# lucasnewman/f5-tts-mlx

Measured on NVIDIA H100. Metric: mel-frames/sec, higher is better.
Workload: dtype bf16

## Files before the change

f5_tts_mlx_b200/csrc/attention.cu:

```cuda
#include "attention_sm90.cuh"
#include "host_common.h"

static int attention_impl(const void* qkv, int64_t ld_qkv, void* out, int64_t ld_out, int32_t batch, int32_t frames,
                          int32_t heads, int32_t head_dim, const int32_t* kv_len, int out_fp8, void* stream_,
                          float* scale_out = nullptr);

extern "C" int f5_attention_fwd(const void* qkv, int64_t ld_qkv, void* out, int64_t ld_out,
                                int32_t batch, int32_t frames, int32_t heads, int32_t head_dim,
                                const int32_t* kv_len, void* stream_) {
  return attention_impl(qkv, ld_qkv, out, ld_out, batch, frames, heads, head_dim, kv_len, 0, stream_);
}
extern "C" int f5_attention_fwd_e4m3(const void* qkv, int64_t ld_qkv, void* out, int64_t ld_out,
                                     int32_t batch, int32_t frames, int32_t heads, int32_t head_dim,
                                     const int32_t* kv_len, void* stream_) {
  return attention_impl(qkv, ld_qkv, out, ld_out, batch, frames, heads, head_dim, kv_len, 1, stream_);
}
extern "C" int f5_attention_fwd_e4m3_scaled(const void* qkv, int64_t ld_qkv, void* out, int64_t ld_out,
                                            int32_t batch, int32_t frames, int32_t heads, int32_t head_dim,
                                            const int32_t* kv_len, float* scale_out, void* stream_) {
  F5_REQUIRE(scale_out != nullptr, "f5_attention_fwd_e4m3_scaled: null scale_out");
  return attention_impl(qkv, ld_qkv, out, ld_out, batch, frames, heads, head_dim, kv_len, 1, stream_, scale_out);
}

static int attention_impl(const void* qkv, int64_t ld_qkv, void* out, int64_t ld_out, int32_t batch, int32_t frames,
                          int32_t heads, int32_t head_dim, const int32_t* kv_len, int out_fp8, void* stream_,
                          float* scale_out) {
  using namespace f5;
  if (int e = device_check()) return e;
  F5_REQUIRE(qkv && out, "f5_attention_fwd: null pointer");
  F5_REQUIRE(head_dim == 64, "f5_attention_fwd: head_dim %d unsupported (only 64)", head_dim);
  F5_REQUIRE(batch > 0 && frames > 0 && heads > 0, "f5_attention_fwd: bad shape");
  F5_REQUIRE(ld_qkv % 8 == 0 && ld_qkv >= 3 * heads * 64, "f5_attention_fwd: bad ld_qkv");
  F5_REQUIRE(ld_out % (out_fp8 ? 16 : 8) == 0 && ld_out >= heads * 64, "f5_attention_fwd: bad ld_out");
  CUtensorMap tm;
  uint64_t dims[3] = {(uint64_t)3 * heads * 64, (uint64_t)frames, (uint64_t)batch};
  uint64_t str[2] = {(uint64_t)ld_qkv * 2, (uint64_t)ld_qkv * 2 * (uint64_t)frames};
  uint32_t box[3] = {64, 128, 1};
  if (int e = make_tmap_bf16(&tm, qkv, 3, dims, str, box)) return e;
  AttnParams p;
  p.B = batch; p.N = frames; p.H = heads;
  p.kv_len = kv_len;
  p.out = reinterpret_cast<__nv_bfloat16*>(out);
  p.ldo = (int)ld_out;
  p.out_fp8 = out_fp8;
  p.scale_out = scale_out;
  cudaStream_t stream = reinterpret_cast<cudaStream_t>(stream_);
  ProfScope ps(PROF_ATTN, 4.0 * batch * heads * (double)frames * frames * 64.0,
               2.0 * batch * (double)frames * heads * 64.0 * 4.0);
  p.prof = ps.slot;
  auto launch = [&](auto kern, SmemAttrOnce& once, dim3 grid, int threads, int smem) -> int {
    F5_CHECK_CUDA(ensure_dyn_smem(once, kern, smem));
    F5_CHECK_CUDA(launch_kernel(kern, grid, dim3(threads), smem, stream, tm, p));
    F5_CHECK_CUDA(cudaGetLastError());
    return 0;
  };
  const dim3 grid(cdiv(frames, 128), heads, batch);
  static SmemAttrOnce o4, o8, o8s;
  if (scale_out != nullptr) return launch(attn_fwd_kernel<true, true>, o8s, grid, 384, AttnSmem::kTotal);
  if (out_fp8) return launch(attn_fwd_kernel<true>, o8, grid, 384, AttnSmem::kTotal);
  return launch(attn_fwd_kernel<false>, o4, grid, 384, AttnSmem::kTotal);
}
```

f5_tts_mlx_b200/csrc/attention_sm90.cuh:

```cuda
#pragma once
#include "ptx.cuh"

namespace f5 {

struct AttnParams {
  int B, N, H;
  const int* kv_len;
  __nv_bfloat16* out;
  int ldo;
  unsigned long long* prof;
  int out_fp8;
  float* scale_out;
};

struct AttnSmem {
  static constexpr int kQ = 0;
  static constexpr int kK = 16384;
  static constexpr int kV = kK + 2 * 16384;
  static constexpr int kBar = kV + 2 * 16384;
  static constexpr int kNumBars = 9;
  static constexpr int kTotal = kBar + kNumBars * 8 + 1024;
};

template <bool kOut8, bool kScaled = false>
__global__ void __launch_bounds__(384, 1)
attn_fwd_kernel(const __grid_constant__ CUtensorMap tma_qkv, const AttnParams p) {
  extern __shared__ uint8_t smem_raw[];
  uint8_t* smem = smem_raw + ((1024u - (smem_u32(smem_raw) & 1023u)) & 1023u);
  uint64_t* bars = reinterpret_cast<uint64_t*>(smem + AttnSmem::kBar);
  uint64_t* q_full = bars + 0;
  uint64_t* k_full = bars + 1;
  uint64_t* k_empty = bars + 3;
  uint64_t* v_full = bars + 5;
  uint64_t* v_empty = bars + 7;

  const int warp = threadIdx.x >> 5, lane = threadIdx.x & 31;
  const int q0 = blockIdx.x * 128;
  const int h = blockIdx.y;
  const int b = blockIdx.z;
  const int HD = p.H * 64;

  if (warp == 0 && elect_one()) {
    tma_prefetch_desc(&tma_qkv);
    mbar_init(q_full, 1);
    for (int i = 0; i < 2; ++i) {
      mbar_init(&k_full[i], 1);
      mbar_init(&k_empty[i], 256);
      mbar_init(&v_full[i], 1);
      mbar_init(&v_empty[i], 256);
    }
    fence_mbar_init();
  }
  __syncthreads();
  pdl_wait();
  if (threadIdx.x == 128) prof_stamp_begin(p.prof);
  int kv_len = p.kv_len ? p.kv_len[b] : p.N;
  kv_len = min(max(kv_len, 1), p.N);
  const int num_kv = (kv_len + 127) >> 7;

  if (warp < 4) {
    if (warp == 0 && elect_one()) {
      mbar_expect_tx(q_full, 16384);
      tma_load_3d(smem + AttnSmem::kQ, &tma_qkv, q_full, h * 64, q0, b);
      for (int j = 0; j < num_kv; ++j) {
        const int s = j & 1;
        const uint32_t ph = (j >> 1) & 1;
        mbar_wait(&k_empty[s], ph ^ 1);
        mbar_expect_tx(&k_full[s], 16384);
        tma_load_3d(smem + AttnSmem::kK + s * 16384, &tma_qkv, &k_full[s], HD + h * 64, j * 128, b);
        mbar_wait(&v_empty[s], ph ^ 1);
        mbar_expect_tx(&v_full[s], 16384);
        tma_load_3d(smem + AttnSmem::kV + s * 16384, &tma_qkv, &v_full[s], 2 * HD + h * 64, j * 128, b);
      }
    }
  } else {
    const int wg = (threadIdx.x >> 7) - 1;
    const int rw = ((threadIdx.x >> 5) & 3) * 16 + (lane >> 2);
    const uint32_t sQ = smem_u32(smem + AttnSmem::kQ) + wg * (64 * 128);
    constexpr float kLog2e = 1.4426950408889634f;
    float o[32];
#pragma unroll
    for (int i = 0; i < 32; ++i) o[i] = 0.f;
    float m_run[2] = {-INFINITY, -INFINITY}, l_run[2] = {0.f, 0.f};
    mbar_wait(q_full, 0);

    for (int j = 0; j < num_kv; ++j) {
      const int s = j & 1;
      const uint32_t ph = (j >> 1) & 1;
      float sv[64];
      mbar_wait(&k_full[s], ph);
      const uint32_t sK = smem_u32(smem + AttnSmem::kK + s * 16384);
      wgmma_fence();
#pragma unroll
      for (int k = 0; k < 4; ++k)
        wgmma_bf16_ss_n128(sv, gmma_desc_sw128(sQ + 32 * k, 16, 1024), gmma_desc_sw128(sK + 32 * k, 16, 1024), k != 0);
      wgmma_commit();
      wgmma_wait<0>();
      wgmma_reg_fence(sv);
      mbar_arrive(&k_empty[s]);

      const int kv0 = j * 128;
      if (kv0 + 128 > kv_len) {
#pragma unroll
        for (int i = 0; i < 64; ++i)
          if (kv0 + 8 * (i >> 2) + 2 * (lane & 3) + (i & 1) >= kv_len) sv[i] = -INFINITY;
      }
      float mx[2] = {m_run[0], m_run[1]};
#pragma unroll
      for (int i = 0; i < 64; ++i) mx[(i >> 1) & 1] = fmaxf(mx[(i >> 1) & 1], sv[i]);
#pragma unroll
      for (int r = 0; r < 2; ++r) {
        mx[r] = fmaxf(mx[r], __shfl_xor_sync(0xffffffffu, mx[r], 1));
        mx[r] = fmaxf(mx[r], __shfl_xor_sync(0xffffffffu, mx[r], 2));
      }
      float sc[2], mb[2];
#pragma unroll
      for (int r = 0; r < 2; ++r) {
        sc[r] = ex2_approx((m_run[r] - mx[r]) * kLog2e);
        m_run[r] = mx[r];
        mb[r] = mx[r] * kLog2e;
        l_run[r] *= sc[r];
      }
#pragma unroll
      for (int i = 0; i < 32; ++i) o[i] *= sc[(i >> 1) & 1];
      uint32_t pa[8][4];
#pragma unroll
      for (int kk = 0; kk < 8; ++kk) {
#pragma unroll
        for (int m = 0; m < 4; ++m) {
          const int i = 8 * kk + 2 * m, r = m & 1;
          const float e0 = ex2_approx(fmaf(sv[i], kLog2e, -mb[r]));
          const float e1 = ex2_approx(fmaf(sv[i + 1], kLog2e, -mb[r]));
          l_run[r] += e0 + e1;
          pa[kk][m] = pack_bf16x2(e0, e1);
        }
      }

      mbar_wait(&v_full[s], ph);
      const uint32_t sV = smem_u32(smem + AttnSmem::kV + s * 16384);
      wgmma_fence();
#pragma unroll
      for (int kk = 0; kk < 8; ++kk) wgmma_bf16_rs_n64_tb(o, pa[kk], gmma_desc_sw128(sV + kk * 2048, 16384, 1024));
      wgmma_commit();
      wgmma_wait<0>();
      wgmma_reg_fence(o);
      mbar_arrive(&v_empty[s]);
    }

    pdl_launch_dependents();
#pragma unroll
    for (int r = 0; r < 2; ++r) {
      l_run[r] += __shfl_xor_sync(0xffffffffu, l_run[r], 1);
      l_run[r] += __shfl_xor_sync(0xffffffffu, l_run[r], 2);
    }
    const float inv[2] = {1.f / l_run[0], 1.f / l_run[1]};
    float qs[2] = {1.f, 1.f}, qinv[2] = {1.f, 1.f};
    if constexpr (kScaled) {
#pragma unroll
      for (int r = 0; r < 2; ++r) {
        float amax = 0.f;
#pragma unroll
        for (int c = 0; c < 8; ++c)
          amax = fmax_nan(amax, fmax_nan(fabsf(o[4 * c + 2 * r] * inv[r]), fabsf(o[4 * c + 2 * r + 1] * inv[r])));
        amax = fmax_nan(amax, __shfl_xor_sync(0xffffffffu, amax, 1));
        amax = fmax_nan(amax, __shfl_xor_sync(0xffffffffu, amax, 2));
        qs[r] = e4m3_block_scale(amax, qinv[r]);
      }
    }
#pragma unroll
    for (int r = 0; r < 2; ++r) {
      const int n = q0 + wg * 64 + rw + 8 * r;
      if (n >= p.N) continue;
      const size_t row = (size_t)b * p.N + n;
      if (kScaled && (lane & 3) == 0) p.scale_out[(size_t)h * p.B * p.N + row] = qs[r];
#pragma unroll
      for (int c = 0; c < 8; ++c) {
        const int col = h * 64 + 8 * c + 2 * (lane & 3);
        float v0 = o[4 * c + 2 * r] * inv[r], v1 = o[4 * c + 2 * r + 1] * inv[r];
        if constexpr (kScaled) { v0 *= qinv[r]; v1 *= qinv[r]; }
        if constexpr (kOut8) {
          uint16_t w;
          asm("cvt.rn.satfinite.e4m3x2.f32 %0, %1, %2;" : "=h"(w) : "f"(v1), "f"(v0));
          *reinterpret_cast<uint16_t*>(reinterpret_cast<uint8_t*>(p.out) + row * p.ldo + col) = w;
        } else {
          *reinterpret_cast<uint32_t*>(p.out + row * p.ldo + col) = pack_bf16x2(v0, v1);
        }
      }
    }
  }

  __syncthreads();
  if (threadIdx.x == 0) prof_stamp_end(p.prof);
}

}
```

f5_tts_mlx_b200/csrc/host_common.h:

```cpp
#pragma once
#include <cuda.h>
#include <cuda_runtime.h>
#include <stdarg.h>
#include <stdint.h>
#include <stdio.h>

#include "../../include/f5_b200.h"

namespace f5 {

int set_error(int code, const char* fmt, ...);

#define F5_CHECK_CUDA(expr)                                                              \
  do {                                                                                   \
    cudaError_t _e = (expr);                                                             \
    if (_e != cudaSuccess)                                                               \
      return f5::set_error(F5_ERR_CUDA, "%s failed: %s (%s:%d)", #expr,                  \
                           cudaGetErrorString(_e), __FILE__, __LINE__);                  \
  } while (0)

#define F5_REQUIRE(cond, ...)                                        \
  do {                                                               \
    if (!(cond)) return f5::set_error(F5_ERR_INVALID, __VA_ARGS__);  \
  } while (0)

int device_check();

int make_tmap_bf16(CUtensorMap* map, const void* base, int rank, const uint64_t* dims,
                   const uint64_t* strides_bytes, const uint32_t* box);
int make_tmap_u8(CUtensorMap* map, const void* base, int rank, const uint64_t* dims,
                 const uint64_t* strides_bytes, const uint32_t* box);
int make_tmap_u8_sw64(CUtensorMap* map, const void* base, int rank, const uint64_t* dims,
                      const uint64_t* strides_bytes, const uint32_t* box);
int make_tmap_out(CUtensorMap* map, const void* base, int elem_bytes, uint64_t cols, uint64_t rows, uint64_t batches,
                  uint64_t ld_elems);

inline int cdiv(int a, int b) { return (a + b - 1) / b; }

int sm_count();

template <typename... KArgs, typename... Args>
inline cudaError_t launch_kernel(void (*kern)(KArgs...), dim3 grid, dim3 block, size_t smem,
                                 cudaStream_t st, Args&&... args) {
  cudaLaunchConfig_t cfg = {};
  cfg.gridDim = grid;
  cfg.blockDim = block;
  cfg.dynamicSmemBytes = smem;
  cfg.stream = st;
  cudaLaunchAttribute attr[1];
  attr[0].id = cudaLaunchAttributeProgrammaticStreamSerialization;
  attr[0].val.programmaticStreamSerializationAllowed = 1;
  cfg.attrs = attr;
  cfg.numAttrs = 1;
  return cudaLaunchKernelEx(&cfg, kern, static_cast<KArgs>(args)...);
}

struct SmemAttrOnce {
  unsigned long long done = 0;
};
template <typename K>
inline cudaError_t ensure_dyn_smem(SmemAttrOnce& once, K kern, int bytes) {
  int dev = 0;
  cudaError_t e = cudaGetDevice(&dev);
  if (e != cudaSuccess) return e;
  if (dev < 64 && ((once.done >> dev) & 1ull)) return cudaSuccess;
  e = cudaFuncSetAttribute(kern, cudaFuncAttributeMaxDynamicSharedMemorySize, bytes);
  if (e == cudaSuccess && dev < 64) once.done |= 1ull << dev;
  return e;
}

enum ProfKind { PROF_GEMM = 0, PROF_ATTN = 1, PROF_LN = 2, PROF_OTHER = 3, PROF_NKINDS = 4 };
struct ProfScope {
  ProfScope(int kind, double flops, double bytes);
  unsigned long long* slot;
};

}
```

f5_tts_mlx_b200/csrc/ptx.cuh:

```cuda
#pragma once
#include <cuda.h>
#include <cuda_runtime.h>
#include <cuda_bf16.h>
#include <stdint.h>
#include <stdio.h>

namespace f5 {

__device__ __forceinline__ uint32_t smem_u32(const void* p) {
  return static_cast<uint32_t>(__cvta_generic_to_shared(p));
}

__device__ __forceinline__ bool elect_one() {
  uint32_t pred = 0;
  asm volatile(
      "{\n\t.reg .pred P;\n\t"
      "elect.sync _|P, 0xffffffff;\n\t"
      "selp.u32 %0, 1, 0, P;\n\t}\n"
      : "=r"(pred));
  return pred != 0;
}

__device__ __forceinline__ void pdl_wait() { asm volatile("griddepcontrol.wait;\n" ::: "memory"); }
__device__ __forceinline__ void pdl_launch_dependents() {
  asm volatile("griddepcontrol.launch_dependents;\n" ::: "memory");
}

__device__ __forceinline__ void prof_stamp_begin(unsigned long long* slot) {
  if (slot != nullptr) {
    unsigned long long t;
    asm volatile("mov.u64 %0, %%globaltimer;" : "=l"(t));
    atomicMin(slot, t);
  }
}
__device__ __forceinline__ void prof_stamp_end(unsigned long long* slot) {
  if (slot != nullptr) {
    unsigned long long t;
    asm volatile("mov.u64 %0, %%globaltimer;" : "=l"(t));
    atomicMax(slot + 1, t);
  }
}

__device__ __forceinline__ void mbar_init(uint64_t* bar, uint32_t count) {
  asm volatile("mbarrier.init.shared::cta.b64 [%0], %1;\n" ::"r"(smem_u32(bar)), "r"(count));
}
__device__ __forceinline__ void fence_mbar_init() {
  asm volatile("fence.mbarrier_init.release.cluster;\n" ::: "memory");
}
__device__ __forceinline__ void fence_proxy_async_smem() {
  asm volatile("fence.proxy.async.shared::cta;\n" ::: "memory");
}
__device__ __forceinline__ void mbar_expect_tx(uint64_t* bar, uint32_t bytes) {
  asm volatile("mbarrier.arrive.expect_tx.shared::cta.b64 _, [%0], %1;\n" ::"r"(smem_u32(bar)),
               "r"(bytes)
               : "memory");
}
__device__ __forceinline__ void mbar_arrive(uint64_t* bar) {
  asm volatile("mbarrier.arrive.shared::cta.b64 _, [%0];\n" ::"r"(smem_u32(bar)) : "memory");
}
__device__ __forceinline__ bool mbar_try_wait(uint64_t* bar, uint32_t parity) {
  uint32_t ok;
  asm volatile(
      "{\n\t.reg .pred P;\n\t"
      "mbarrier.try_wait.parity.shared::cta.b64 P, [%1], %2;\n\t"
      "selp.u32 %0, 1, 0, P;\n\t}\n"
      : "=r"(ok)
      : "r"(smem_u32(bar)), "r"(parity)
      : "memory");
  return ok != 0;
}
__device__ __forceinline__ void mbar_wait(uint64_t* bar, uint32_t parity) {
  if (mbar_try_wait(bar, parity)) return;
  const long long t0 = clock64();
  uint32_t spins = 0;
  while (!mbar_try_wait(bar, parity)) {
    if ((++spins & 0x3ff) == 0 && (clock64() - t0) > 4000000000LL) asm volatile("trap;");
  }
}

__device__ __forceinline__ void tma_prefetch_desc(const CUtensorMap* m) {
  asm volatile("prefetch.tensormap [%0];\n" ::"l"(m) : "memory");
}
__device__ __forceinline__ void tma_load_2d(void* smem_dst, const CUtensorMap* m, uint64_t* bar,
                                            int c0, int c1) {
  asm volatile(
      "cp.async.bulk.tensor.2d.shared::cluster.global.mbarrier::complete_tx::bytes"
      " [%0], [%1, {%3, %4}], [%2];\n" ::"r"(smem_u32(smem_dst)),
      "l"(m), "r"(smem_u32(bar)), "r"(c0), "r"(c1)
      : "memory");
}
__device__ __forceinline__ void tma_load_3d(void* smem_dst, const CUtensorMap* m, uint64_t* bar,
                                            int c0, int c1, int c2) {
  asm volatile(
      "cp.async.bulk.tensor.3d.shared::cluster.global.mbarrier::complete_tx::bytes"
      " [%0], [%1, {%3, %4, %5}], [%2];\n" ::"r"(smem_u32(smem_dst)),
      "l"(m), "r"(smem_u32(bar)), "r"(c0), "r"(c1), "r"(c2)
      : "memory");
}
__device__ __forceinline__ void tma_load_4d(void* smem_dst, const CUtensorMap* m, uint64_t* bar,
                                            int c0, int c1, int c2, int c3) {
  asm volatile(
      "cp.async.bulk.tensor.4d.shared::cluster.global.mbarrier::complete_tx::bytes"
      " [%0], [%1, {%3, %4, %5, %6}], [%2];\n" ::"r"(smem_u32(smem_dst)),
      "l"(m), "r"(smem_u32(bar)), "r"(c0), "r"(c1), "r"(c2), "r"(c3)
      : "memory");
}

__device__ __forceinline__ void tma_store_3d(const CUtensorMap* m, const void* smem_src, int c0, int c1, int c2) {
  asm volatile("cp.async.bulk.tensor.3d.global.shared::cta.bulk_group [%0, {%2, %3, %4}], [%1];\n" ::"l"(m),
               "r"(smem_u32(smem_src)), "r"(c0), "r"(c1), "r"(c2)
               : "memory");
}
__device__ __forceinline__ void tma_store_commit() { asm volatile("cp.async.bulk.commit_group;\n" ::: "memory"); }
template <int N>
__device__ __forceinline__ void tma_store_wait_read() {
  asm volatile("cp.async.bulk.wait_group.read %0;\n" ::"n"(N) : "memory");
}
template <int N>
__device__ __forceinline__ void tma_store_wait() {
  asm volatile("cp.async.bulk.wait_group %0;\n" ::"n"(N) : "memory");
}

__device__ __forceinline__ void wgmma_fence() { asm volatile("wgmma.fence.sync.aligned;\n" ::: "memory"); }
__device__ __forceinline__ void wgmma_commit() { asm volatile("wgmma.commit_group.sync.aligned;\n" ::: "memory"); }
template <int N>
__device__ __forceinline__ void wgmma_wait() {
  asm volatile("wgmma.wait_group.sync.aligned %0;\n" ::"n"(N) : "memory");
}
template <int N>
__device__ __forceinline__ void wgmma_reg_fence(float (&d)[N]) {
#pragma unroll
  for (int i = 0; i < N; ++i) asm volatile("" : "+f"(d[i])::"memory");
}

__host__ __device__ constexpr uint64_t gmma_desc_sw128(uint32_t saddr, uint32_t lbo_bytes, uint32_t sbo_bytes) {
  return (uint64_t)((saddr >> 4) & 0x3FFF) | ((uint64_t)((lbo_bytes >> 4) & 0x3FFF) << 16) |
         ((uint64_t)((sbo_bytes >> 4) & 0x3FFF) << 32) | ((uint64_t)1 << 62);
}
__host__ __device__ constexpr uint64_t gmma_desc_sw64(uint32_t saddr, uint32_t lbo_bytes, uint32_t sbo_bytes) {
  return (uint64_t)((saddr >> 4) & 0x3FFF) | ((uint64_t)((lbo_bytes >> 4) & 0x3FFF) << 16) |
         ((uint64_t)((sbo_bytes >> 4) & 0x3FFF) << 32) | ((uint64_t)2 << 62);
}

__device__ __forceinline__ void wgmma_bf16_ss_n64(float (&d)[32], uint64_t desc_a, uint64_t desc_b, uint32_t scale_d) {
  asm volatile(
      "{\n\t.reg .pred p;\n\tsetp.ne.b32 p, %34, 0;\n\t"
      "wgmma.mma_async.sync.aligned.m64n64k16.f32.bf16.bf16 "
      "{%0, %1, %2, %3, %4, %5, %6, %7, %8, %9, %10, %11, %12, %13, %14, %15, %16, %17, %18, %19, %20, %21, %22, %23, %24, %25, %26, %27, %28, %29, %30, %31}, %32, %33, p, 1, 1, 0, 0;\n\t}\n"
      : "+f"(d[0]), "+f"(d[1]), "+f"(d[2]), "+f"(d[3]), "+f"(d[4]), "+f"(d[5]), "+f"(d[6]), "+f"(d[7]), "+f"(d[8]), "+f"(d[9]), "+f"(d[10]), "+f"(d[11]), "+f"(d[12]), "+f"(d[13]), "+f"(d[14]), "+f"(d[15]), "+f"(d[16]), "+f"(d[17]), "+f"(d[18]), "+f"(d[19]), "+f"(d[20]), "+f"(d[21]), "+f"(d[22]), "+f"(d[23]), "+f"(d[24]), "+f"(d[25]), "+f"(d[26]), "+f"(d[27]), "+f"(d[28]), "+f"(d[29]), "+f"(d[30]), "+f"(d[31])
      : "l"(desc_a), "l"(desc_b), "r"(scale_d));
}
__device__ __forceinline__ void wgmma_bf16_ss_n128(float (&d)[64], uint64_t desc_a, uint64_t desc_b, uint32_t scale_d) {
  asm volatile(
      "{\n\t.reg .pred p;\n\tsetp.ne.b32 p, %66, 0;\n\t"
      "wgmma.mma_async.sync.aligned.m64n128k16.f32.bf16.bf16 "
      "{%0, %1, %2, %3, %4, %5, %6, %7, %8, %9, %10, %11, %12, %13, %14, %15, %16, %17, %18, %19, %20, %21, %22, %23, %24, %25, %26, %27, %28, %29, %30, %31, %32, %33, %34, %35, %36, %37, %38, %39, %40, %41, %42, %43, %44, %45, %46, %47, %48, %49, %50, %51, %52, %53, %54, %55, %56, %57, %58, %59, %60, %61, %62, %63}, %64, %65, p, 1, 1, 0, 0;\n\t}\n"
      : "+f"(d[0]), "+f"(d[1]), "+f"(d[2]), "+f"(d[3]), "+f"(d[4]), "+f"(d[5]), "+f"(d[6]), "+f"(d[7]), "+f"(d[8]), "+f"(d[9]), "+f"(d[10]), "+f"(d[11]), "+f"(d[12]), "+f"(d[13]), "+f"(d[14]), "+f"(d[15]), "+f"(d[16]), "+f"(d[17]), "+f"(d[18]), "+f"(d[19]), "+f"(d[20]), "+f"(d[21]), "+f"(d[22]), "+f"(d[23]), "+f"(d[24]), "+f"(d[25]), "+f"(d[26]), "+f"(d[27]), "+f"(d[28]), "+f"(d[29]), "+f"(d[30]), "+f"(d[31]), "+f"(d[32]), "+f"(d[33]), "+f"(d[34]), "+f"(d[35]), "+f"(d[36]), "+f"(d[37]), "+f"(d[38]), "+f"(d[39]), "+f"(d[40]), "+f"(d[41]), "+f"(d[42]), "+f"(d[43]), "+f"(d[44]), "+f"(d[45]), "+f"(d[46]), "+f"(d[47]), "+f"(d[48]), "+f"(d[49]), "+f"(d[50]), "+f"(d[51]), "+f"(d[52]), "+f"(d[53]), "+f"(d[54]), "+f"(d[55]), "+f"(d[56]), "+f"(d[57]), "+f"(d[58]), "+f"(d[59]), "+f"(d[60]), "+f"(d[61]), "+f"(d[62]), "+f"(d[63])
      : "l"(desc_a), "l"(desc_b), "r"(scale_d));
}
__device__ __forceinline__ void wgmma_e4m3_ss_n64(float (&d)[32], uint64_t desc_a, uint64_t desc_b, uint32_t scale_d) {
  asm volatile(
      "{\n\t.reg .pred p;\n\tsetp.ne.b32 p, %34, 0;\n\t"
      "wgmma.mma_async.sync.aligned.m64n64k32.f32.e4m3.e4m3 "
      "{%0, %1, %2, %3, %4, %5, %6, %7, %8, %9, %10, %11, %12, %13, %14, %15, %16, %17, %18, %19, %20, %21, %22, %23, %24, %25, %26, %27, %28, %29, %30, %31}, %32, %33, p, 1, 1;\n\t}\n"
      : "+f"(d[0]), "+f"(d[1]), "+f"(d[2]), "+f"(d[3]), "+f"(d[4]), "+f"(d[5]), "+f"(d[6]), "+f"(d[7]), "+f"(d[8]), "+f"(d[9]), "+f"(d[10]), "+f"(d[11]), "+f"(d[12]), "+f"(d[13]), "+f"(d[14]), "+f"(d[15]), "+f"(d[16]), "+f"(d[17]), "+f"(d[18]), "+f"(d[19]), "+f"(d[20]), "+f"(d[21]), "+f"(d[22]), "+f"(d[23]), "+f"(d[24]), "+f"(d[25]), "+f"(d[26]), "+f"(d[27]), "+f"(d[28]), "+f"(d[29]), "+f"(d[30]), "+f"(d[31])
      : "l"(desc_a), "l"(desc_b), "r"(scale_d));
}
__device__ __forceinline__ void wgmma_e4m3_ss_n128(float (&d)[64], uint64_t desc_a, uint64_t desc_b, uint32_t scale_d) {
  asm volatile(
      "{\n\t.reg .pred p;\n\tsetp.ne.b32 p, %66, 0;\n\t"
      "wgmma.mma_async.sync.aligned.m64n128k32.f32.e4m3.e4m3 "
      "{%0, %1, %2, %3, %4, %5, %6, %7, %8, %9, %10, %11, %12, %13, %14, %15, %16, %17, %18, %19, %20, %21, %22, %23, %24, %25, %26, %27, %28, %29, %30, %31, %32, %33, %34, %35, %36, %37, %38, %39, %40, %41, %42, %43, %44, %45, %46, %47, %48, %49, %50, %51, %52, %53, %54, %55, %56, %57, %58, %59, %60, %61, %62, %63}, %64, %65, p, 1, 1;\n\t}\n"
      : "+f"(d[0]), "+f"(d[1]), "+f"(d[2]), "+f"(d[3]), "+f"(d[4]), "+f"(d[5]), "+f"(d[6]), "+f"(d[7]), "+f"(d[8]), "+f"(d[9]), "+f"(d[10]), "+f"(d[11]), "+f"(d[12]), "+f"(d[13]), "+f"(d[14]), "+f"(d[15]), "+f"(d[16]), "+f"(d[17]), "+f"(d[18]), "+f"(d[19]), "+f"(d[20]), "+f"(d[21]), "+f"(d[22]), "+f"(d[23]), "+f"(d[24]), "+f"(d[25]), "+f"(d[26]), "+f"(d[27]), "+f"(d[28]), "+f"(d[29]), "+f"(d[30]), "+f"(d[31]), "+f"(d[32]), "+f"(d[33]), "+f"(d[34]), "+f"(d[35]), "+f"(d[36]), "+f"(d[37]), "+f"(d[38]), "+f"(d[39]), "+f"(d[40]), "+f"(d[41]), "+f"(d[42]), "+f"(d[43]), "+f"(d[44]), "+f"(d[45]), "+f"(d[46]), "+f"(d[47]), "+f"(d[48]), "+f"(d[49]), "+f"(d[50]), "+f"(d[51]), "+f"(d[52]), "+f"(d[53]), "+f"(d[54]), "+f"(d[55]), "+f"(d[56]), "+f"(d[57]), "+f"(d[58]), "+f"(d[59]), "+f"(d[60]), "+f"(d[61]), "+f"(d[62]), "+f"(d[63])
      : "l"(desc_a), "l"(desc_b), "r"(scale_d));
}
__device__ __forceinline__ void wgmma_bf16_rs_n64_tb(float (&d)[32], const uint32_t (&a)[4], uint64_t desc_b) {
  asm volatile(
      "{\n\t.reg .pred p;\n\tsetp.ne.b32 p, 1, 0;\n\t"
      "wgmma.mma_async.sync.aligned.m64n64k16.f32.bf16.bf16 "
      "{%0, %1, %2, %3, %4, %5, %6, %7, %8, %9, %10, %11, %12, %13, %14, %15, %16, %17, %18, %19, %20, %21, %22, %23, %24, %25, %26, %27, %28, %29, %30, %31}, {%32, %33, %34, %35}, %36, p, 1, 1, 1;\n\t}\n"
      : "+f"(d[0]), "+f"(d[1]), "+f"(d[2]), "+f"(d[3]), "+f"(d[4]), "+f"(d[5]), "+f"(d[6]), "+f"(d[7]), "+f"(d[8]), "+f"(d[9]), "+f"(d[10]), "+f"(d[11]), "+f"(d[12]), "+f"(d[13]), "+f"(d[14]), "+f"(d[15]), "+f"(d[16]), "+f"(d[17]), "+f"(d[18]), "+f"(d[19]), "+f"(d[20]), "+f"(d[21]), "+f"(d[22]), "+f"(d[23]), "+f"(d[24]), "+f"(d[25]), "+f"(d[26]), "+f"(d[27]), "+f"(d[28]), "+f"(d[29]), "+f"(d[30]), "+f"(d[31])
      : "r"(a[0]), "r"(a[1]), "r"(a[2]), "r"(a[3]), "l"(desc_b));
}
__device__ __forceinline__ void wgmma_e4m3_rs_n64(float (&d)[32], const uint32_t (&a)[4], uint64_t desc_b,
                                                  uint32_t scale_d) {
  asm volatile(
      "{\n\t.reg .pred p;\n\tsetp.ne.b32 p, %37, 0;\n\t"
      "wgmma.mma_async.sync.aligned.m64n64k32.f32.e4m3.e4m3 "
      "{%0, %1, %2, %3, %4, %5, %6, %7, %8, %9, %10, %11, %12, %13, %14, %15, %16, %17, %18, %19, %20, %21, %22, %23, %24, %25, %26, %27, %28, %29, %30, %31}, {%32, %33, %34, %35}, %36, p, 1, 1;\n\t}\n"
      : "+f"(d[0]), "+f"(d[1]), "+f"(d[2]), "+f"(d[3]), "+f"(d[4]), "+f"(d[5]), "+f"(d[6]), "+f"(d[7]), "+f"(d[8]), "+f"(d[9]), "+f"(d[10]), "+f"(d[11]), "+f"(d[12]), "+f"(d[13]), "+f"(d[14]), "+f"(d[15]), "+f"(d[16]), "+f"(d[17]), "+f"(d[18]), "+f"(d[19]), "+f"(d[20]), "+f"(d[21]), "+f"(d[22]), "+f"(d[23]), "+f"(d[24]), "+f"(d[25]), "+f"(d[26]), "+f"(d[27]), "+f"(d[28]), "+f"(d[29]), "+f"(d[30]), "+f"(d[31])
      : "r"(a[0]), "r"(a[1]), "r"(a[2]), "r"(a[3]), "l"(desc_b), "r"(scale_d));
}


__device__ __forceinline__ float gelu_tanh_f(float x) {
  const float k0 = 0.7978845608028654f, k1 = 0.044715f;
  float u = k0 * (x + k1 * x * x * x);
  return 0.5f * x * (1.f + tanhf(u));
}
__device__ __forceinline__ float gelu_erf_f(float x) {
  return 0.5f * x * (1.f + erff(x * 0.7071067811865476f));
}
__device__ __forceinline__ float mish_f(float x) {
  float sp = (x > 20.f) ? x : log1pf(expf(x));
  return x * tanhf(sp);
}
__device__ __forceinline__ float silu_f(float x) { return x / (1.f + expf(-x)); }

__device__ __forceinline__ float ex2_approx(float x) {
  float y;
  asm("ex2.approx.ftz.f32 %0, %1;" : "=f"(y) : "f"(x));
  return y;
}

__device__ __forceinline__ uint32_t pack_bf16x2(float lo, float hi) {
  __nv_bfloat162 v = __floats2bfloat162_rn(lo, hi);
  return *reinterpret_cast<uint32_t*>(&v);
}

__device__ __forceinline__ uint32_t pack_e4m3x4(float a, float b, float c, float d) {
  uint16_t lo, hi;
  asm("cvt.rn.satfinite.e4m3x2.f32 %0, %1, %2;" : "=h"(lo) : "f"(b), "f"(a));
  asm("cvt.rn.satfinite.e4m3x2.f32 %0, %1, %2;" : "=h"(hi) : "f"(d), "f"(c));
  return (uint32_t)lo | ((uint32_t)hi << 16);
}

__device__ __forceinline__ float fmax_nan(float a, float b) {
  float y;
  asm("max.NaN.f32 %0, %1, %2;" : "=f"(y) : "f"(a), "f"(b));
  return y;
}

__device__ __forceinline__ float e4m3_block_scale(float amax, float& inv) {
  const uint32_t b = __float_as_uint(amax);
  const int e = (int)(b >> 23) & 0xFF;
  if (e == 0xFF) { inv = 0.f; return amax; }
  if (b == 0u) { inv = 1.f; return 1.f; }
  int k = e - 135 + ((b & 0x7FFFFFu) > 0x600000u ? 1 : 0);
  k = k < -126 ? -126 : k;
  inv = __uint_as_float((uint32_t)(127 - k) << 23);
  return __uint_as_float((uint32_t)(k + 127) << 23);
}

}
```

Measured before the change: 10890.

## Drop producer warpgroup so two attention CTAs fit per SM

Removes the dedicated TMA producer warpgroup, shrinking the attention CTA to 256 threads with launch bounds allowing two CTAs per SM and max shared-memory carveout. Consumers now release K/V buffers by counting arrivals with shared atomics, and the last arriving warp issues the next TMA load itself, replacing the empty mbarriers. The PV wgmma is split into two batches so the first half can issue before all P values are packed. Tail CTAs with fewer than 64 valid rows use a single consumer warpgroup. A test hook reporting achieved CTAs per SM is added; the risk is register pressure at the tighter launch bounds and load latency now sitting on the consumers' critical path.

```diff
diff --git a/f5_tts_mlx_b200/csrc/attention.cu b/f5_tts_mlx_b200/csrc/attention.cu
--- a/f5_tts_mlx_b200/csrc/attention.cu
+++ b/f5_tts_mlx_b200/csrc/attention.cu
@@ -1,5 +1,19 @@
 #include "attention_sm90.cuh"
 #include "host_common.h"
+
+static f5::SmemAttrOnce g_attn_attrs[3];
+
+template <typename F>
+static int with_attn_kernel(int form, F&& f) {
+  using namespace f5;
+  auto go = [&](auto kern) -> int {
+    F5_CHECK_CUDA(ensure_dyn_smem(g_attn_attrs[form], kern, AttnSmem::kTotal, true));
+    return f(kern);
+  };
+  if (form == 2) return go(attn_fwd_kernel<true, true>);
+  if (form == 1) return go(attn_fwd_kernel<true, false>);
+  return go(attn_fwd_kernel<false, false>);
+}
 
 static int attention_impl(const void* qkv, int64_t ld_qkv, void* out, int64_t ld_out, int32_t batch, int32_t frames,
                           int32_t heads, int32_t head_dim, const int32_t* kv_len, int out_fp8, void* stream_,
@@ -48,15 +62,20 @@
   ProfScope ps(PROF_ATTN, 4.0 * batch * heads * (double)frames * frames * 64.0,
                2.0 * batch * (double)frames * heads * 64.0 * 4.0);
   p.prof = ps.slot;
-  auto launch = [&](auto kern, SmemAttrOnce& once, dim3 grid, int threads, int smem) -> int {
-    F5_CHECK_CUDA(ensure_dyn_smem(once, kern, smem));
-    F5_CHECK_CUDA(launch_kernel(kern, grid, dim3(threads), smem, stream, tm, p));
+  const dim3 grid(cdiv(frames, 128), heads, batch);
+  return with_attn_kernel(scale_out != nullptr ? 2 : out_fp8 ? 1 : 0, [&](auto kern) -> int {
+    F5_CHECK_CUDA(launch_kernel(kern, grid, dim3(kAttnThreads), AttnSmem::kTotal, stream, tm, p));
     F5_CHECK_CUDA(cudaGetLastError());
     return 0;
-  };
-  const dim3 grid(cdiv(frames, 128), heads, batch);
-  static SmemAttrOnce o4, o8, o8s;
-  if (scale_out != nullptr) return launch(attn_fwd_kernel<true, true>, o8s, grid, 384, AttnSmem::kTotal);
-  if (out_fp8) return launch(attn_fwd_kernel<true>, o8, grid, 384, AttnSmem::kTotal);
-  return launch(attn_fwd_kernel<false>, o4, grid, 384, AttnSmem::kTotal);
+  });
 }
+
+extern "C" int f5_attention_test_ctas_per_sm(int form) {
+  if (int e = f5::device_check()) return e;
+  F5_REQUIRE(form >= 0 && form <= 2, "f5_attention_test_ctas_per_sm: bad form %d", form);
+  return with_attn_kernel(form, [](auto kern) -> int {
+    int n = 0;
+    F5_CHECK_CUDA(cudaOccupancyMaxActiveBlocksPerMultiprocessor(&n, kern, f5::kAttnThreads, f5::AttnSmem::kTotal));
+    return n;
+  });
+}
diff --git a/f5_tts_mlx_b200/csrc/attention_sm90.cuh b/f5_tts_mlx_b200/csrc/attention_sm90.cuh
--- a/f5_tts_mlx_b200/csrc/attention_sm90.cuh
+++ b/f5_tts_mlx_b200/csrc/attention_sm90.cuh
@@ -18,65 +18,72 @@
   static constexpr int kK = 16384;
   static constexpr int kV = kK + 2 * 16384;
   static constexpr int kBar = kV + 2 * 16384;
-  static constexpr int kNumBars = 9;
-  static constexpr int kTotal = kBar + kNumBars * 8 + 1024;
+  static constexpr int kNumBars = 5;
+  static constexpr int kRel = kBar + kNumBars * 8;
+  static constexpr int kTotal = kRel + 4 * 4 + 1024;
 };
+constexpr int kAttnThreads = 256;
+static_assert(2 * (AttnSmem::kTotal + 1024) <= 228 * 1024, "attn_fwd_kernel no longer fits twice per SM");
 
 template <bool kOut8, bool kScaled = false>
-__global__ void __launch_bounds__(384, 1)
+__global__ void __launch_bounds__(kAttnThreads, 2)
 attn_fwd_kernel(const __grid_constant__ CUtensorMap tma_qkv, const AttnParams p) {
   extern __shared__ uint8_t smem_raw[];
   uint8_t* smem = smem_raw + ((1024u - (smem_u32(smem_raw) & 1023u)) & 1023u);
   uint64_t* bars = reinterpret_cast<uint64_t*>(smem + AttnSmem::kBar);
   uint64_t* q_full = bars + 0;
   uint64_t* k_full = bars + 1;
-  uint64_t* k_empty = bars + 3;
-  uint64_t* v_full = bars + 5;
-  uint64_t* v_empty = bars + 7;
+  uint64_t* v_full = bars + 3;
+  uint32_t* k_rel = reinterpret_cast<uint32_t*>(smem + AttnSmem::kRel);
+  uint32_t* v_rel = k_rel + 2;
 
   const int warp = threadIdx.x >> 5, lane = threadIdx.x & 31;
+  const int wg = threadIdx.x >> 7;
   const int q0 = blockIdx.x * 128;
   const int h = blockIdx.y;
   const int b = blockIdx.z;
   const int HD = p.H * 64;
+  const int nwg = q0 + 64 < p.N ? 2 : 1;
 
   if (warp == 0 && elect_one()) {
     tma_prefetch_desc(&tma_qkv);
     mbar_init(q_full, 1);
     for (int i = 0; i < 2; ++i) {
       mbar_init(&k_full[i], 1);
-      mbar_init(&k_empty[i], 256);
       mbar_init(&v_full[i], 1);
-      mbar_init(&v_empty[i], 256);
+      k_rel[i] = 0;
+      v_rel[i] = 0;
     }
     fence_mbar_init();
   }
   __syncthreads();
   pdl_wait();
-  if (threadIdx.x == 128) prof_stamp_begin(p.prof);
+  if (threadIdx.x == 0) prof_stamp_begin(p.prof);
   int kv_len = p.kv_len ? p.kv_len[b] : p.N;
   kv_len = min(max(kv_len, 1), p.N);
   const int num_kv = (kv_len + 127) >> 7;
 
-  if (warp < 4) {
-    if (warp == 0 && elect_one()) {
-      mbar_expect_tx(q_full, 16384);
-      tma_load_3d(smem + AttnSmem::kQ, &tma_qkv, q_full, h * 64, q0, b);
-      for (int j = 0; j < num_kv; ++j) {
-        const int s = j & 1;
-        const uint32_t ph = (j >> 1) & 1;
-        mbar_wait(&k_empty[s], ph ^ 1);
-        mbar_expect_tx(&k_full[s], 16384);
-        tma_load_3d(smem + AttnSmem::kK + s * 16384, &tma_qkv, &k_full[s], HD + h * 64, j * 128, b);
-        mbar_wait(&v_empty[s], ph ^ 1);
-        mbar_expect_tx(&v_full[s], 16384);
-        tma_load_3d(smem + AttnSmem::kV + s * 16384, &tma_qkv, &v_full[s], 2 * HD + h * 64, j * 128, b);
-      }
-    }
-  } else {
-    const int wg = (threadIdx.x >> 7) - 1;
+  auto load_k = [&](int j) {
+    mbar_expect_tx(&k_full[j & 1], 16384);
+    tma_load_3d(smem + AttnSmem::kK + (j & 1) * 16384, &tma_qkv, &k_full[j & 1], HD + h * 64, j * 128, b);
+  };
+  auto load_v = [&](int j) {
+    mbar_expect_tx(&v_full[j & 1], 16384);
+    tma_load_3d(smem + AttnSmem::kV + (j & 1) * 16384, &tma_qkv, &v_full[j & 1], 2 * HD + h * 64, j * 128, b);
+  };
+  if (warp == 0 && elect_one()) {
+    mbar_expect_tx(q_full, 16384);
+    tma_load_3d(smem + AttnSmem::kQ, &tma_qkv, q_full, h * 64, q0, b);
+    for (int j = 0; j < min(num_kv, 2); ++j) {
+      load_k(j);
+      load_v(j);
+    }
+  }
+
+  if (wg < nwg) {
     const int rw = ((threadIdx.x >> 5) & 3) * 16 + (lane >> 2);
     const uint32_t sQ = smem_u32(smem + AttnSmem::kQ) + wg * (64 * 128);
+    const uint32_t rel_per_use = 4 * nwg;
     constexpr float kLog2e = 1.4426950408889634f;
     float o[32];
 #pragma unroll
@@ -87,6 +94,7 @@
     for (int j = 0; j < num_kv; ++j) {
       const int s = j & 1;
       const uint32_t ph = (j >> 1) & 1;
+      const uint32_t last_rel = ((j >> 1) + 1) * rel_per_use - 1;
       float sv[64];
       mbar_wait(&k_full[s], ph);
       const uint32_t sK = smem_u32(smem + AttnSmem::kK + s * 16384);
@@ -97,7 +105,7 @@
       wgmma_commit();
       wgmma_wait<0>();
       wgmma_reg_fence(sv);
-      mbar_arrive(&k_empty[s]);
+      if (elect_one() && atom_add_acq_rel_smem(&k_rel[s], 1) == last_rel && j + 2 < num_kv) load_k(j + 2);
 
       const int kv0 = j * 128;
       if (kv0 + 128 > kv_len) {
@@ -123,6 +131,8 @@
       }
 #pragma unroll
       for (int i = 0; i < 32; ++i) o[i] *= sc[(i >> 1) & 1];
+
+      const uint32_t sV = smem_u32(smem + AttnSmem::kV + s * 16384);
       uint32_t pa[8][4];
 #pragma unroll
       for (int kk = 0; kk < 8; ++kk) {
@@ -134,17 +144,18 @@
           l_run[r] += e0 + e1;
           pa[kk][m] = pack_bf16x2(e0, e1);
         }
-      }
-
-      mbar_wait(&v_full[s], ph);
-      const uint32_t sV = smem_u32(smem + AttnSmem::kV + s * 16384);
-      wgmma_fence();
-#pragma unroll
-      for (int kk = 0; kk < 8; ++kk) wgmma_bf16_rs_n64_tb(o, pa[kk], gmma_desc_sw128(sV + kk * 2048, 16384, 1024));
+        if ((kk & 3) == 3) {
+          if (kk == 3) mbar_wait(&v_full[s], ph);
+          wgmma_fence();
+#pragma unroll
+          for (int k2 = kk - 3; k2 <= kk; ++k2)
+            wgmma_bf16_rs_n64_tb(o, pa[k2], gmma_desc_sw128(sV + k2 * 2048, 16384, 1024));
+        }
+      }
       wgmma_commit();
       wgmma_wait<0>();
       wgmma_reg_fence(o);
-      mbar_arrive(&v_empty[s]);
+      if (elect_one() && atom_add_acq_rel_smem(&v_rel[s], 1) == last_rel && j + 2 < num_kv) load_v(j + 2);
     }
 
     pdl_launch_dependents();
diff --git a/f5_tts_mlx_b200/csrc/host_common.h b/f5_tts_mlx_b200/csrc/host_common.h
--- a/f5_tts_mlx_b200/csrc/host_common.h
+++ b/f5_tts_mlx_b200/csrc/host_common.h
@@ -59,12 +59,14 @@
   unsigned long long done = 0;
 };
 template <typename K>
-inline cudaError_t ensure_dyn_smem(SmemAttrOnce& once, K kern, int bytes) {
+inline cudaError_t ensure_dyn_smem(SmemAttrOnce& once, K kern, int bytes, bool max_carveout = false) {
   int dev = 0;
   cudaError_t e = cudaGetDevice(&dev);
   if (e != cudaSuccess) return e;
   if (dev < 64 && ((once.done >> dev) & 1ull)) return cudaSuccess;
   e = cudaFuncSetAttribute(kern, cudaFuncAttributeMaxDynamicSharedMemorySize, bytes);
+  if (e == cudaSuccess && max_carveout)
+    e = cudaFuncSetAttribute(kern, cudaFuncAttributePreferredSharedMemoryCarveout, cudaSharedmemCarveoutMaxShared);
   if (e == cudaSuccess && dev < 64) once.done |= 1ull << dev;
   return e;
 }
diff --git a/f5_tts_mlx_b200/csrc/ptx.cuh b/f5_tts_mlx_b200/csrc/ptx.cuh
--- a/f5_tts_mlx_b200/csrc/ptx.cuh
+++ b/f5_tts_mlx_b200/csrc/ptx.cuh
@@ -19,6 +19,12 @@
       "selp.u32 %0, 1, 0, P;\n\t}\n"
       : "=r"(pred));
   return pred != 0;
+}
+
+__device__ __forceinline__ uint32_t atom_add_acq_rel_smem(uint32_t* p, uint32_t v) {
+  uint32_t old;
+  asm volatile("atom.acq_rel.cta.shared::cta.add.u32 %0, [%1], %2;\n" : "=r"(old) : "r"(smem_u32(p)), "r"(v) : "memory");
+  return old;
 }
 
 __device__ __forceinline__ void pdl_wait() { asm volatile("griddepcontrol.wait;\n" ::: "memory"); }
```

Measured after the change: 11140, median of 6. +2.3%, better.
